# ntnu-arl/mimosa

Hardware: AMD Instinct MI355X
Metric: ICP corr+residual Mpts/sec, 131k-pt scan vs 5M-pt map, 1/2/4/8 GPU (higher is better)
Workload: dtype f64; 1 GPU; configs[1]: OS0-128 131072-pt scan vs 4963194-pt local map (511380 voxels, 2x5 rooms), k=5 point-to-plane, ENWIDE params, cold linearize per step; parallelism=single GPU, exact_fallback_queries=0

## Files before the change

mimosa_amd/csrc/icp_device.hpp:

```cpp
#pragma once

#include <hip/hip_runtime.h>

#include <cstdint>
#include <cstring>

#include "flagged_word.hpp"
#include "voxel_map.hpp"

namespace mh
{
constexpr int kPartialStride = 96;

struct MapView
{
  const int4 * table;
  const uint32_t * cells;
  const float4 * buckets;
  const uint4 * qbuckets;
  double inv_leaf;
  uint32_t mask;
  int n_off;
  int mode_idx;
};

struct DeviceResult
{
  double sums[kPartialStride];
  double eig_rot[9], eig_trans[9];
  double loc_comp[6];
  unsigned long long n_knn, n_cand, n_fallback, n_scanned;
  unsigned int status_hist[9];
};

constexpr int kLlSums = 96;
constexpr int kLlEig = 32;
constexpr int kLlRow = 8;
constexpr int kLocChunks = 4;
__host__ __device__ inline size_t ll_slot_words(int loc_grid_cap) { return static_cast<size_t>(kLlSums + kLlEig) + static_cast<size_t>(loc_grid_cap) * kLlRow; }

struct IcpArgs
{
  MapView map;
  const float4 * src;
  int n;
  int k;
  int cold;
  int use_huber;
  double R[9], t[3];
  double da_thresh, max_d2, plane_valid, sigma, huber;
  double inv_sigma;
  double inv_huber;
  double * q_da;
  double * mean;
  double * normal;
  int32_t * status;
  double * partials;
  unsigned int * ticket;
  unsigned int seq;
  int tail;
  uint4 * ll;
  unsigned long long * dbg;
  int reps;
  const uint32_t * n_dev = nullptr;
  double * shard_out = nullptr;
  double * rec = nullptr;
  int rec_n = 0;
};
__host__ __device__ inline size_t loc_record_bytes(size_t n) { return n * (6 * sizeof(double) + sizeof(int32_t)); }
constexpr int32_t kShardSkip = 0x100;

struct LocArgs
{
  unsigned int seq;
  int nv;
  const float4 * src;
  int n;
  int chunks_per_block;
  int k;
  int k3_blocks;
  uint4 * ll;
  double R[9];
  const double * normal;
  const int32_t * status;
  double * partials;
  unsigned int * ticket;
  const uint32_t * n_dev = nullptr;
  const double * sums = nullptr;
  double * shard_out = nullptr;
  const double * rec = nullptr;
  int rec_n = 0;
  unsigned long long * dbg = nullptr;
};

int linearize_class(int n, int k, bool shard, long long total = 0);
int class_grid(int n, int ppw);
int class_loc_grid(int n, int ppw, bool shard = false);
int linearize_grid_max(int n);
hipError_t launch_linearize(const IcpArgs & a, bool binary, hipStream_t stream);
hipError_t launch_localizability(const LocArgs & a, hipStream_t stream);
hipError_t launch_linearize_batch(const IcpArgs * d_args, const int * d_start, int n_factors, int total_grid, int tpb, int k,
                                  int n_off, bool binary, hipStream_t stream);
hipError_t launch_localizability_batch(const LocArgs * d_args, const int * d_start, int n_factors, int total_grid, int tpb,
                                       hipStream_t stream);
constexpr int kBatchInline = 8;
template <typename A>
struct BatchInline
{
  A a[kBatchInline];
  int start[kBatchInline + 1];
  int n;
  char pad[256];
};
template <typename A, typename ArgAt, typename GridAt>
inline int fill_batch_inline(BatchInline<A> & blk, int n, ArgAt && arg_at, GridAt && grid_at)
{
  std::memset(static_cast<void *>(&blk), 0, sizeof(blk));
  int acc = 0;
  for (int i = 0; i < n; ++i) {
    blk.a[i] = arg_at(i);
    blk.start[i] = acc;
    acc += grid_at(i);
  }
  blk.start[n] = acc;
  blk.n = n;
  return acc;
}
hipError_t launch_linearize_batch_inline(const BatchInline<IcpArgs> & blk, int total_grid, int tpb, int k, int n_off, bool binary,
                                         hipStream_t stream, bool shard = false);
hipError_t launch_localizability_batch_inline(const BatchInline<LocArgs> & blk, int total_grid, int tpb, hipStream_t stream, bool shard = false);
hipError_t launch_map_knn(const MapView & map, const double * q, int n, int k, double * pts, double * sq,
                          int32_t * found, hipStream_t stream);

size_t order_temp_bytes(int n);
hipError_t launch_spatial_order(const float4 * xyz_in, int n, float cell, uint32_t * keys2, uint32_t * vals, void * temp,
                                size_t temp_bytes, uint32_t * perm, float4 * xyz_out, hipStream_t stream);
size_t source_order_scratch_bytes(int n);
hipError_t launch_source_order(const mh_point32 * d_pts, int n, float cell, void * scratch, uint32_t * perm, float4 * xyz_out,
                               uint32_t * zero, int n_zero, hipStream_t stream);
hipError_t launch_unpermute_state(const uint32_t * perm, int n, const int32_t * st_in, const double * mean_in,
                                  const double * nrm_in, int32_t * st_out, double * mean_out, double * nrm_out,
                                  hipStream_t stream);

hipError_t launch_deskew(mh_point32 * pts, int n, const uint32_t * unique_ns, const float * Rt12, int n_groups,
// ... 7 lines not shown
```

mimosa_amd/csrc/icp_kernels.hip:

```cpp
#include <hip/hip_runtime.h>

#include <cstdlib>

#include "icp_device.hpp"

#ifndef MH_PRUNE_TRIPS
#define MH_PRUNE_TRIPS (trip == 1 || trip == 2)
#endif
#ifndef MH_PIPE
#define MH_PIPE 4
#endif
#ifndef MH_XCD_PIECES
#define MH_XCD_PIECES 2
#endif
#ifndef MH_PIPE_SMALL
#define MH_PIPE_SMALL 4
#endif
#include "map_device.hpp"
#include "math3.hpp"
#include "wave_dpp.hpp"

namespace mh
{
namespace
// ... 860 lines not shown
  jt[1] = -ns1;
  jt[2] = -ns2;
}

template <int K, bool BINARY, int NOFF, int TPB, bool SHARD, int QL = 1>
__device__ __forceinline__ void icp_linearize_body(const IcpArgs & a, const int block_id, const int n_blocks)
{
  static_assert(QL == 1 || (!SHARD && K == 5), "several lanes per query: plain k = 5 factors only");
  constexpr int PPW = TPB / QL;
  [[maybe_unused]] const bool lead = QL == 1 || (threadIdx.x & static_cast<unsigned int>(QL - 1)) == 0u;
  constexpr int NV = BINARY ? 13 : 7;
  constexpr int NENT = NV * (NV + 1) / 2;
  constexpr int EW = BINARY ? 96 : 32;
  constexpr int ROWW = NV;
  constexpr int kListWords = NOFF * PPW;
  constexpr int kFoldWords = (TPB / EW) * EW * 2 + EW * 2;
  constexpr int kArenaWords = kListWords > kFoldWords ? kListWords : kFoldWords;
  __shared__ __attribute__((aligned(16))) uint32_t s_arena[kArenaWords];
  __shared__ double s_tile[TPB * ROWW];
  __shared__ double s_wsum[(TPB / 64) * (NENT <= 32 ? 2 : 1) * NENT];
  __shared__ unsigned int s_cnt[4];
  __shared__ uint32_t s_scan[kScanLutWords];
  __shared__ bool s_last;

  uint32_t * s_list = s_arena + threadIdx.x / QL;
  double * s_aux = reinterpret_cast<double *>(s_arena);

#if !defined(MH_NO_INTERLEAVE)
  const int qi = [&] {
    if constexpr (QL > 1) return xcd_chunk(block_id, n_blocks) * PPW + static_cast<int>(threadIdx.x) / QL;
    constexpr int WPB = TPB / 64;
    const int cpx = n_blocks >> 3, x = block_id & 7, j = block_id >> 3, wv = static_cast<int>(threadIdx.x >> 6);
#if MH_XCD_PIECES > 1
    constexpr int P = MH_XCD_PIECES;
    static_assert(WPB % P == 0, "pieces must divide the waves of a workgroup");
    const int S = cpx * (WPB / P), p = wv / (WPB / P), o = (wv % (WPB / P)) * cpx + j;
    return ((p * 8 + ((p & 1) ? 7 - x : x)) * S + o) * 64 + static_cast<int>(threadIdx.x & 63u);
#else
    return ((x * cpx * WPB) + wv * cpx + j) * 64 + static_cast<int>(threadIdx.x & 63u);
#endif
  }();
#else
  const int qi = xcd_chunk(block_id, n_blocks) * PPW + static_cast<int>(threadIdx.x) / QL;
#endif
  const int k = (K == 5) ? 5 : a.k;
  const int n_pts = SHARD ? static_cast<int>(*a.n_dev) : a.n;
  float4 sp = make_float4(0.f, 0.f, 0.f, 0.f);
  if (qi < n_pts) sp = a.src[qi];
  if (threadIdx.x < 4) s_cnt[threadIdx.x] = 0u;
  fill_scan_lut<NOFF>(s_scan);
  __syncthreads();

  double row[NV];
  [[maybe_unused]] double rec_jr[3] = {0.0, 0.0, 0.0}, rec_jt[3] = {0.0, 0.0, 0.0};
  [[maybe_unused]] int rec_st = -1;
  uint32_t cnt_pack = 0u;
  bool did_knn = false, did_fall = false;
#ifdef MH_TIMELINE
  for (int rep = 0; rep < a.reps; ++rep) {
  if (rep > 0) {
    __syncthreads();
    if (threadIdx.x < 4) s_cnt[threadIdx.x] = 0u;
    __syncthreads();
  }
#endif
  MH_STAMP(a.dbg, 0);
#pragma unroll
  for (int j = 0; j < NV; ++j) row[j] = 0.0;

  if (qi < n_pts) {
    const double px = sp.x, py = sp.y, pz = sp.z;
    const double q0 = (a.R[0] * px + (a.R[1] * py + a.R[2] * pz)) + a.t[0];
    const double q1 = (a.R[3] * px + (a.R[4] * py + a.R[5] * pz)) + a.t[1];
    const double q2 = (a.R[6] * px + (a.R[7] * py + a.R[8] * pz)) + a.t[2];

    double qd0 = 0.0, qd1 = 0.0, qd2 = 0.0;
    int st = MH_UNPROCESSED;
    if (!a.cold) {
      qd0 = a.q_da[3 * qi + 0];
      qd1 = a.q_da[3 * qi + 1];
      qd2 = a.q_da[3 * qi + 2];
      st = a.status[qi];
    }
    bool gone = SHARD && (st & kShardSkip) != 0;
    if constexpr (SHARD) {
      if (a.cold) {
        const int raw = a.status[qi];
        gone = (raw & kShardSkip) != 0;
        if (gone && raw != -1) {
          a.status[qi] = kShardSkip;
          a.q_da[3 * qi + 0] = a.q_da[3 * qi + 1] = a.q_da[3 * qi + 2] = 0.0;
          a.mean[3 * qi + 0] = a.mean[3 * qi + 1] = a.mean[3 * qi + 2] = 0.0;
          a.normal[3 * qi + 0] = a.normal[3 * qi + 1] = a.normal[3 * qi + 2] = 0.0;
        }
      }
    }
    const double ddx = q0 - qd0, ddy = q1 - qd1, ddz = q2 - qd2;
    const bool update = !gone && (ddx * ddx + (ddy * ddy + ddz * ddz)) > a.da_thresh * a.da_thresh;

    double mean[3] = {0, 0, 0}, nrm[3] = {0, 0, 0};
    bool go = false;
    if (update) {
      st = MH_UNPROCESSED;
      if (lead) {
        a.q_da[3 * qi + 0] = q0;
        a.q_da[3 * qi + 1] = q1;
        a.q_da[3 * qi + 2] = q2;
      }
// ... 126 lines not shown
      }
    } else {
      if (!gone && st > MH_CORRES_PLANE_INVALID) {
        mean[0] = a.mean[3 * qi + 0];
        mean[1] = a.mean[3 * qi + 1];
        mean[2] = a.mean[3 * qi + 2];
        nrm[0] = a.normal[3 * qi + 0];
        nrm[1] = a.normal[3 * qi + 1];
        nrm[2] = a.normal[3 * qi + 2];
        go = true;
      } else if (a.cold && lead) {
        a.q_da[3 * qi + 0] = a.q_da[3 * qi + 1] = a.q_da[3 * qi + 2] = 0.0;
        a.mean[3 * qi + 0] = a.mean[3 * qi + 1] = a.mean[3 * qi + 2] = 0.0;
        a.normal[3 * qi + 0] = a.normal[3 * qi + 1] = a.normal[3 * qi + 2] = 0.0;
      }
    }

    if (go && lead) {
      double e = nrm[0] * (mean[0] - q0) + (nrm[1] * (mean[1] - q1) + nrm[2] * (mean[2] - q2));
      const double r2 = px * px + (py * py + pz * pz);
      const double e81 = 81.0 * (e * e);
      if (e81 * e81 > r2) {
        st = MH_MAX_ERROR;
      } else {
        double sw = 1.0;
        if (a.use_huber) {
          const double we = e * a.inv_sigma;
          if (fabs(we) > a.huber) sw = mh_rsqrt(fabs(we) * a.inv_huber);
        }
        const double wgt = sw * a.inv_sigma;
        e *= wgt;
        const double ns0 = a.R[0] * nrm[0] + (a.R[3] * nrm[1] + a.R[6] * nrm[2]);
        const double ns1 = a.R[1] * nrm[0] + (a.R[4] * nrm[1] + a.R[7] * nrm[2]);
        const double ns2 = a.R[2] * nrm[0] + (a.R[5] * nrm[1] + a.R[8] * nrm[2]);
        row[0] = (ns1 * pz - ns2 * py) * wgt;
        row[1] = (ns2 * px - ns0 * pz) * wgt;
        row[2] = (ns0 * py - ns1 * px) * wgt;
        row[3] = -ns0 * wgt;
        row[4] = -ns1 * wgt;
        row[5] = -ns2 * wgt;
        if constexpr (BINARY) {
          row[6] = (q1 * nrm[2] - q2 * nrm[1]) * wgt;
          row[7] = (q2 * nrm[0] - q0 * nrm[2]) * wgt;
          row[8] = (q0 * nrm[1] - q1 * nrm[0]) * wgt;
          row[9] = nrm[0] * wgt;
          row[10] = nrm[1] * wgt;
          row[11] = nrm[2] * wgt;
        }
        row[NV - 1] = e;
        st = MH_VALID;
      }
    }
    if (!gone && lead) a.status[qi] = st;
    if constexpr (!SHARD) {
      if (a.rec && lead) {
        if (st == MH_VALID) loc_directions(a, nrm[0], nrm[1], nrm[2], px, py, pz, rec_jr, rec_jt);
        rec_st = st;
      }
    }
  }
  {
    const uint32_t packed = wave_sum_to_lane63(cnt_pack);
    const unsigned long long mk = __ballot(did_knn), mf = __ballot(did_fall);
    if ((threadIdx.x & 63) == 63) {
      atomicAdd(&s_cnt[0], static_cast<unsigned int>(__popcll(mk)));
      atomicAdd(&s_cnt[1], packed & 0xFFFFu);
      atomicAdd(&s_cnt[2], static_cast<unsigned int>(__popcll(mf)));
      atomicAdd(&s_cnt[3], packed >> 16);
    }
    cnt_pack = 0u;
    did_knn = did_fall = false;
  }
#ifdef MH_TIMELINE
  }
#endif

  [[maybe_unused]] auto store_record = [&]() {
    if constexpr (!SHARD) {
      const size_t rn = static_cast<size_t>(a.rec_n);
      int32_t * rst = reinterpret_cast<int32_t *>(a.rec + 6 * rn);
#pragma unroll
      for (int c = 0; c < 3; ++c) {
        a.rec[static_cast<size_t>(c) * rn + qi] = rec_jr[c];
        a.rec[static_cast<size_t>(3 + c) * rn + qi] = rec_jt[c];
      }
      rst[qi] = rec_st;
    }
  };
  MH_STAMP(a.dbg, 3);
  {
    constexpr int WSEG = NENT <= 32 ? 2 : 1;
    constexpr int WPTS = 64 / WSEG;
    const int lane = static_cast<int>(threadIdx.x & 63u), wv = static_cast<int>(threadIdx.x >> 6);
    double * tile = s_tile + static_cast<size_t>(wv) * 64 * ROWW;
#pragma unroll
    for (int j = 0; j < NV; ++j) tile[lane * ROWW + j] = row[j];
    __builtin_amdgcn_fence(__ATOMIC_RELEASE, "wavefront");
    __builtin_amdgcn_wave_barrier();
    __builtin_amdgcn_fence(__ATOMIC_ACQUIRE, "wavefront");
    constexpr int ROUNDS = (NENT * WSEG + 63) / 64;
#pragma unroll
    for (int rd = 0; rd < ROUNDS; ++rd) {
      const int item = rd * 64 + lane;
      const int ent = WSEG == 2 ? (lane & 31) : item, seg = WSEG == 2 ? (lane >> 5) : 0;
      if (ent < NENT) {
        int r = 0, rem = ent;
        while (rem >= NV - r) {
          rem -= NV - r;
          ++r;
        }
        const int c = r + rem;
        const double * pr = tile + seg * WPTS * ROWW;
        double s0 = 0.0, s1 = 0.0, s2 = 0.0, s3 = 0.0;
#pragma unroll
        for (int p = 0; p < WPTS; p += 4) {
          s0 += pr[(p + 0) * ROWW + r] * pr[(p + 0) * ROWW + c];
          s1 += pr[(p + 1) * ROWW + r] * pr[(p + 1) * ROWW + c];
          s2 += pr[(p + 2) * ROWW + r] * pr[(p + 2) * ROWW + c];
          s3 += pr[(p + 3) * ROWW + r] * pr[(p + 3) * ROWW + c];
        }
        s_wsum[(wv * WSEG + seg) * NENT + ent] = (s0 + s1) + (s2 + s3);
      }
    }
    if constexpr (!SHARD) {
      if (a.rec && qi < a.n && lead) store_record();
    }
  }
  __syncthreads();
  MH_STAMP(a.dbg, 4);
  const bool fold_here = SHARD || a.tail != 0;
  const bool through = fold_here;
  if (threadIdx.x < NENT) {
    constexpr int NPART = (TPB / 64) * (NENT <= 32 ? 2 : 1);
    double pv[NPART];
#pragma unroll
    for (int g = 0; g < NPART; ++g) pv[g] = s_wsum[g * NENT + threadIdx.x];
    double s = 0.0;
#pragma unroll
    for (int g = 0; g < NPART; ++g) s += pv[g];
    double * dst = &a.partials[static_cast<size_t>(block_id) * kPartialStride + threadIdx.x];
    if (through)
      store_partial(dst, s);
    else
      *dst = s;
  }
  if (threadIdx.x >= 128 && threadIdx.x < 132) {
    double * dst = &a.partials[static_cast<size_t>(block_id) * kPartialStride + NENT + (threadIdx.x - 128)];
    const double c = static_cast<double>(s_cnt[threadIdx.x - 128]);
    if (through)
      store_partial(dst, c);
    else
      *dst = c;
  }

  MH_STAMP(a.dbg, 5);
  if (!fold_here) return;
  if (!arrive_is_last(a.ticket, static_cast<unsigned int>(n_blocks), &s_last)) return;
  MH_STAMP(a.dbg, 6);

  double * s_sum = s_aux + (TPB / EW) * EW;
  fold_rows<EW, TPB>(a.partials, n_blocks, NENT + 4, s_aux, s_sum);
  if constexpr (SHARD) {
    if (threadIdx.x < NENT + 4) a.shard_out[threadIdx.x] = s_sum[threadIdx.x];
  } else {
    if (threadIdx.x < NENT + 4) ll_store(a.ll + threadIdx.x, s_sum[threadIdx.x], a.seq);
  }
  MH_STAMP(a.dbg, 7);
}

template <int K, bool BINARY, int NOFF, int TPB, bool SHARD, int QL = 1>
__global__ __launch_bounds__(TPB) void icp_linearize_kernel(const IcpArgs a)
{
  icp_linearize_body<K, BINARY, NOFF, TPB, SHARD, QL>(a, static_cast<int>(blockIdx.x), static_cast<int>(gridDim.x));
}

template <typename T>
__device__ __forceinline__ T load_uniform(const T * p)
{
  static_assert(sizeof(T) % 4 == 0, "dword-sized argument blocks only");
// ... 4 lines not shown
    __device__ U() {}
  } u;
  const uint32_t * s = reinterpret_cast<const uint32_t *>(p);
  const int lane = static_cast<int>(threadIdx.x & 63u);
  uint32_t chunk[NL];
#pragma unroll
  for (int c = 0; c < NL; ++c) chunk[c] = s[c * 64 + lane];
#pragma unroll
  for (int i = 0; i < NW; ++i) u.w[i] = static_cast<uint32_t>(__builtin_amdgcn_readlane(static_cast<int>(chunk[i / 64]), i % 64));
  return u.v;
}

__device__ __forceinline__ int batch_factor_of(const int * start, int n_factors, int b)
{
  int f = 0;
  for (int i = 1; i < n_factors; ++i) f += (b >= start[i]) ? 1 : 0;
  return __builtin_amdgcn_readfirstlane(f);
}

template <int K, bool BINARY, int NOFF, int TPB>
__global__ __launch_bounds__(TPB) void icp_linearize_batch_kernel(const IcpArgs * args, const int * start, int n_factors)
{
  const int b = static_cast<int>(blockIdx.x);
  const int f = batch_factor_of(start, n_factors, b);
  const int s0 = __builtin_amdgcn_readfirstlane(start[f]), s1 = __builtin_amdgcn_readfirstlane(start[f + 1]);
  const IcpArgs a = load_uniform(args + f);
  icp_linearize_body<K, BINARY, NOFF, TPB, false>(a, b - s0, s1 - s0);
}

template <int NOFF, int QL>
__global__ __launch_bounds__(256) void icp_linearize_batch_ql_kernel(const IcpArgs * args, const int * start, int n_factors)
{
  const int b = static_cast<int>(blockIdx.x);
  const int f = batch_factor_of(start, n_factors, b);
  const int s0 = __builtin_amdgcn_readfirstlane(start[f]), s1 = __builtin_amdgcn_readfirstlane(start[f + 1]);
  const IcpArgs a = load_uniform(args + f);
  icp_linearize_body<5, false, NOFF, 256, false, QL>(a, b - s0, s1 - s0);
}

template <int K, bool BINARY, int NOFF, int TPB, bool SHARD, int QL = 1>
__global__ __launch_bounds__(TPB) void icp_linearize_batch_inline_kernel(const BatchInline<IcpArgs> blk)
{
  (void)blk;
  const auto * p = (const BatchInline<IcpArgs> *)__builtin_amdgcn_kernarg_segment_ptr();
  const int b = static_cast<int>(blockIdx.x);
  const int f = batch_factor_of(p->start, p->n, b);
  const int s0 = __builtin_amdgcn_readfirstlane(p->start[f]), s1 = __builtin_amdgcn_readfirstlane(p->start[f + 1]);
  const IcpArgs a = load_uniform(p->a + f);
  icp_linearize_body<K, BINARY, NOFF, TPB, SHARD, QL>(a, b - s0, s1 - s0);
}

__host__ __device__ constexpr int loc_tpb(int tpb, bool shard) { return (!shard && tpb > 256) ? 256 : tpb; }
__host__ __device__ constexpr int loc_threads(int tpb, bool shard) { return loc_tpb(tpb, shard) + (shard ? 0 : 64); }
#ifndef MH_LOC_BLOCKS_512
#define MH_LOC_BLOCKS_512 2
#endif
__host__ __device__ constexpr int loc_ch(int tpb, bool shard) { return shard ? 1 : (tpb > 256 ? 2 * MH_LOC_BLOCKS_512 : kLocChunks); }

template <int TPB, bool SHARD, int CH, bool XW = false>
__device__ __forceinline__ void icp_localizability_body(const LocArgs & a, const int block_id, const int n_blocks)
{
  constexpr int NW = TPB / 64;
  const bool worker = !XW || threadIdx.x < static_cast<unsigned int>(TPB);
  __shared__ double s_w[NW][16];
  __shared__ double s_seg[TPB + 96 + 96];

  const int lane = threadIdx.x & 63, wv = threadIdx.x >> 6;
  MH_STAMP4(a.dbg, 0);
  double v[6] = {0, 0, 0, 0, 0, 0};
  unsigned long long hpack = 0ull;
  const int n_pts = !worker ? 0 : (SHARD ? static_cast<int>(*a.n_dev) : (a.rec ? a.n : 0));
  int st_c[CH];
  double jr_c[CH][3], jt_c[CH][3];
  [[maybe_unused]] float4 sp_c[CH];
  [[maybe_unused]] double nx_c[CH], ny_c[CH], nz_c[CH];
  auto load_chunk = [&](const int ch) {
    const int i = (block_id * CH + ch) * TPB + static_cast<int>(threadIdx.x);
    const int i_ld = i < n_pts ? i : 0;
    st_c[ch] = -1;
    jr_c[ch][0] = jr_c[ch][1] = jr_c[ch][2] = jt_c[ch][0] = jt_c[ch][1] = jt_c[ch][2] = 0.0;
    if constexpr (SHARD) {
      sp_c[ch] = make_float4(0.f, 0.f, 0.f, 0.f);
      nx_c[ch] = ny_c[ch] = nz_c[ch] = 0.0;
      if (n_pts > 0) {
        st_c[ch] = a.status[i_ld];
        sp_c[ch] = a.src[i_ld];
        nx_c[ch] = a.normal[3 * i_ld];
        ny_c[ch] = a.normal[3 * i_ld + 1];
        nz_c[ch] = a.normal[3 * i_ld + 2];
      }
    } else if (n_pts > 0) {
      const size_t rn = static_cast<size_t>(a.rec_n);
      const int32_t * rst = reinterpret_cast<const int32_t *>(a.rec + 6 * rn);
      st_c[ch] = rst[i_ld];
#pragma unroll
      for (int c = 0; c < 3; ++c) {
        jr_c[ch][c] = a.rec[static_cast<size_t>(c) * rn + i_ld];
        jt_c[ch][c] = a.rec[static_cast<size_t>(3 + c) * rn + i_ld];
      }
    }
    if (i >= n_pts) st_c[ch] = -1;
  };
  auto load_all = [&]() {
    MH_STAMP4(a.dbg, 1);
#pragma unroll
    for (int ch = 0; ch < CH; ++ch) load_chunk(ch);
  };
  const double * sums = nullptr;
  double * s_h = s_seg + TPB;
  if constexpr (SHARD) {
    sums = a.sums;
  } else {
    const int n_ent = a.nv * (a.nv + 1) / 2 + 4;
    constexpr int FB = 32;
    if (a.nv == 7)
      fold_rows<32, TPB, true, FB>(a.partials, a.k3_blocks, n_ent, s_seg, s_h);
    else
      fold_rows<96, TPB, true, FB>(a.partials, a.k3_blocks, n_ent, s_seg, s_h);
    sums = s_h;
  }
  load_all();
  MH_STAMP4(a.dbg, 2);
  __shared__ double s_E[18];
  if (XW ? (threadIdx.x == TPB || threadIdx.x == TPB + 1) : (threadIdx.x == TPB - 64 || threadIdx.x == TPB - 128)) {
    const int NV = a.nv, o = (XW ? threadIdx.x == TPB + 1 : threadIdx.x == TPB - 64) ? 3 : 0;
    double Hb[9];
    for (int r = 0; r < 3; ++r)
      for (int c = 0; c < 3; ++c) {
        const int rr = (r < c ? r : c) + o, cc = (r < c ? c : r) + o;
        Hb[3 * r + c] = sums[rr * NV - rr * (rr - 1) / 2 + (cc - rr)];
      }
    double loc[3], E[9];
    if (!sym_eigvec3_fast(Hb, E)) compute_localizability(Hb, loc, E);
    for (int q = 0; q < 9; ++q) s_E[(o ? 9 : 0) + q] = E[q];
  }
  MH_STAMP4(a.dbg, 3);
  if constexpr (SHARD) {
#pragma unroll
    for (int ch = 0; ch < CH; ++ch)
      loc_directions(a, nx_c[ch], ny_c[ch], nz_c[ch], static_cast<double>(sp_c[ch].x), static_cast<double>(sp_c[ch].y),
                     static_cast<double>(sp_c[ch].z), jr_c[ch], jt_c[ch]);
  }
  MH_STAMP4(a.dbg, 4);
  __syncthreads();
  MH_STAMP4(a.dbg, 5);
  double er[9], et[9];
#pragma unroll
  for (int q = 0; q < 9; ++q) {
    er[q] = s_E[q];
    et[q] = s_E[9 + q];
  }
#pragma unroll
  for (int ch = 0; ch < CH; ++ch) {
    const int st = st_c[ch];
    if (st == MH_VALID) {
#pragma unroll
      for (int c = 0; c < 3; ++c) {
        const double tc = fabs(jt_c[ch][0] * et[c] + (jt_c[ch][1] * et[3 + c] + jt_c[ch][2] * et[6 + c]));
        const double rc = fabs(jr_c[ch][0] * er[c] + (jr_c[ch][1] * er[3 + c] + jr_c[ch][2] * er[6 + c]));
        v[c] += tc >= 0.5 ? tc : 0.0;
        v[3 + c] += rc >= 0.5 ? rc : 0.0;
      }
    }
    hpack += st >= 0 && st < 9 ? (1ull << (4 * st)) : 0ull;
  }
  MH_STAMP4(a.dbg, 6);
  wave_sum6_f64_to_lane63(v);
  uint32_t hw[3];
#pragma unroll
  for (int g = 0; g < 3; ++g) {
    const uint32_t f0 = static_cast<uint32_t>(hpack >> (12 * g)) & 15u, f1 = static_cast<uint32_t>(hpack >> (12 * g + 4)) & 15u,
                   f2 = static_cast<uint32_t>(hpack >> (12 * g + 8)) & 15u;
    hw[g] = f0 | (f1 << 10) | (f2 << 20);
  }
  wave_sum3_to_lane63(hw);
  if (lane == 63 && worker) {
#pragma unroll
    for (int j = 0; j < 6; ++j) s_w[wv][j] = v[j];
#pragma unroll
    for (int g = 0; g < 3; ++g) {
      s_w[wv][6 + 3 * g + 0] = static_cast<double>(hw[g] & 1023u);
      s_w[wv][6 + 3 * g + 1] = static_cast<double>((hw[g] >> 10) & 1023u);
      s_w[wv][6 + 3 * g + 2] = static_cast<double>((hw[g] >> 20) & 1023u);
    }
  }
  MH_STAMP4(a.dbg, 7);
  __syncthreads();
  MH_STAMP4(a.dbg, 8);
  if constexpr (!SHARD) {
    uint4 * ll_rows = a.ll + (kLlSums + kLlEig) + static_cast<size_t>(block_id) * kLlRow;
    if (threadIdx.x < 6) {
      double s = 0.0;
      for (int w2 = 0; w2 < NW; ++w2) s += s_w[w2][threadIdx.x];
      ll_store(ll_rows + threadIdx.x, s, a.seq);
    } else if (threadIdx.x < 8) {
      const int h0 = threadIdx.x == 6 ? 0 : 5, hn = threadIdx.x == 6 ? 5 : 4;
      unsigned long long pk = 0ull;
      for (int h = 0; h < hn; ++h) {
        unsigned int c = 0u;
        for (int w2 = 0; w2 < NW; ++w2) c += static_cast<unsigned int>(s_w[w2][6 + h0 + h]);
        pk |= static_cast<unsigned long long>(c) << (12 * h);
      }
      ll_store_bits(ll_rows + threadIdx.x, pk, a.seq);
    }
    if (block_id == 0) {
      const int n_ent = a.nv * (a.nv + 1) / 2 + 4;
      if (threadIdx.x >= 64 && static_cast<int>(threadIdx.x) < 64 + n_ent) ll_store(a.ll + (threadIdx.x - 64), s_h[threadIdx.x - 64], a.seq);
      if (threadIdx.x >= 192 && threadIdx.x < 192 + 18) ll_store(a.ll + kLlSums + (threadIdx.x - 192), s_E[threadIdx.x - 192], a.seq);
    }
#ifdef MH_TIMELINE
    asm volatile("s_waitcnt vmcnt(0)" ::: "memory");
#endif
// ... 349 lines not shown
```

mimosa_amd/csrc/mh_api.hip:

```cpp
#include <hip/hip_runtime.h>

#include <atomic>
#include <cmath>
#include <cstdio>
#include <cstdlib>
#include <cstring>
#include <ctime>
#include <mutex>
#include <new>
#include <unordered_map>
#include <string>
#include <vector>

#include "../../include/mimosa_hip.h"
#include "align_device.hpp"
#include "icp_device.hpp"
#include "math3.hpp"
#include "mh_internal.hpp"
#include "scan_device.hpp"
#include "shard_device.hpp"
#include "voxel_map.hpp"

namespace
{
// ... 427 lines not shown
{
  if (!src || !out) return fail(src ? src->ctx : nullptr, MH_ERR_INVALID_ARG, "mh_icp_clone: NULL argument");
  *out = nullptr;
  mh_ctx * ctx = src->ctx;
  if (src->n_pending) return fail(ctx, MH_ERR_INVALID_ARG, "mh_icp_clone: source has linearize calls in flight");
  MH_HIP(ctx, mh_enter(ctx));
  mh_icp * icp = new (std::nothrow) mh_icp;
  if (!icp) return fail(ctx, MH_ERR_OOM, "mh_icp_clone: host allocation failed");
  icp->ctx = ctx;
  icp->map = src->map;
  mh_map_retain(icp->map);
  map_add_reader(icp->map, ctx);
  icp->n = src->n;
  icp->cfg = src->cfg;
  icp->binary = src->binary;
  int rc = icp_alloc(icp);
  if (rc != MH_OK) {
    mh_icp_destroy(icp);
    return rc;
  }
  const size_t n = src->n;
  auto cp = [&](const DevBuf & a, DevBuf & b, size_t bytes) {
    return bytes ? hipMemcpyAsync(b.p, a.p, bytes, hipMemcpyDeviceToDevice, ctx->stream) : hipSuccess;
  };
  MH_HIP(ctx, cp(src->d_src, icp->d_src, n * sizeof(float4)));
  MH_HIP(ctx, cp(src->d_qda, icp->d_qda, n * 3 * sizeof(double)));
  MH_HIP(ctx, cp(src->d_mean, icp->d_mean, n * 3 * sizeof(double)));
  MH_HIP(ctx, cp(src->d_normal, icp->d_normal, n * 3 * sizeof(double)));
  MH_HIP(ctx, cp(src->d_status, icp->d_status, n * sizeof(int32_t)));
  if (src->ordered) {
    MH_HIP(ctx, icp->d_perm.reserve(n * sizeof(uint32_t), ctx->stream, false));
    MH_HIP(ctx, cp(src->d_perm, icp->d_perm, n * sizeof(uint32_t)));
    icp->ordered = true;
  }
  MH_HIP(ctx, hipMemsetAsync(icp->d_ticket.p, 0, 2 * sizeof(unsigned int), ctx->stream));
  MH_HIP(ctx, hipStreamSynchronize(ctx->stream));
  icp->cold = src->cold;
  icp->components = src->components;
  icp->linearize_count = src->linearize_count;
  *out = icp;
  return MH_OK;
}
int mh_icp_clone(const mh_icp * src, mh_icp ** out)
{
  return guarded(src ? src->ctx : nullptr, "mh_icp_clone", [&]() -> int { return mh_icp_clone_impl(src, out); });
}

void mh_icp_destroy(mh_icp * icp)
{
  if (!icp) return;
  (void)mh_enter(icp->ctx);
  (void)hipStreamSynchronize(icp->ctx->stream);
  if (icp->in_window && icp->ctx->window.active) window_release(icp->ctx);
  icp->d_rec.release(true);
  icp->d_src.release(true);
  icp->d_qda.release(true);
  icp->d_mean.release(true);
  icp->d_normal.release(true);
  icp->d_status.release(true);
  icp->d_partials.release(true);
  icp->d_ticket.release(true);
  icp->d_dbg.release(true);
  icp->d_perm.release(true);
  for (DevBuf * b : {&icp->d_origin, &icp->x_src, &icp->x_qda, &icp->x_mean, &icp->x_normal, &icp->x_status, &icp->x_origin, &icp->s_keys_a,
                     &icp->s_keys_b, &icp->s_idx_a, &icp->s_idx_b, &icp->s_counts, &icp->s_temp, &icp->d_sums})
    b->release(true);
  if (icp->h_counts) (void)hipHostFree(icp->h_counts);
  if (icp->h_ll) AllocCache::free_pinned(icp->h_ll, icp->ll_words * sizeof(uint4) * kMaxPending);
  icp->d_align.release(true);
  if (icp->h_align) AllocCache::free_pinned(icp->h_align, kAlignStageBytes);
  if (icp->events_ready)
    for (auto & ev : icp->events)
      for (auto & e : ev) (void)hipEventDestroy(e);
  if (icp->map) {
    map_remove_reader(icp->map, icp->ctx);
    mh_map_release(icp->map);
  }
  delete icp;
}

size_t mh_icp_size(const mh_icp * icp) { return icp ? icp->n : 0; }

#ifdef MH_TIMELINE
int mh_icp_timeline(mh_icp * icp, unsigned long long * out, size_t capacity_words, size_t * n_words)
{
  if (!icp || !out || !n_words) return MH_ERR_INVALID_ARG;
  mh_ctx * ctx = icp->ctx;
  const size_t words = 2 * static_cast<size_t>(mh::linearize_grid_max(static_cast<int>(icp->n))) * 8 * 16;
  *n_words = words;
  if (capacity_words < words) return MH_ERR_INVALID_ARG;
  MH_HIP(ctx, mh_enter(ctx));
  MH_HIP(ctx, hipStreamSynchronize(ctx->stream));
  MH_HIP(ctx, hipMemcpy(out, icp->d_dbg.p, words * sizeof(unsigned long long), hipMemcpyDeviceToHost));
  return MH_OK;
}
#endif

static int mh_icp_reset_impl(mh_icp * icp)
{
  if (!icp) return fail(nullptr, MH_ERR_INVALID_ARG, "mh_icp_reset: icp is NULL");
  if (icp->in_window) return fail(icp->ctx, MH_ERR_INVALID_ARG, "mh_icp_reset: the factor is in a window call in flight");
  if (icp->align.active) return fail(icp->ctx, MH_ERR_INVALID_ARG, "mh_icp_reset: an alignment is in flight");
  icp->cold = true;
  return MH_OK;
}
int mh_icp_reset(mh_icp * icp)
{
// ... 15 lines not shown
struct LinearizeTxn
{
  mh_icp * icp;
  bool cold = true, committed = false;
  int count = 0, pending = 0;
  explicit LinearizeTxn(mh_icp * i) : icp(i)
  {
    if (icp) {
      cold = icp->cold;
      count = icp->linearize_count;
      pending = icp->n_pending;
    }
  }
  LinearizeTxn(LinearizeTxn && o) noexcept : icp(o.icp), cold(o.cold), committed(o.committed), count(o.count), pending(o.pending) { o.icp = nullptr; }
  LinearizeTxn(const LinearizeTxn &) = delete;
  LinearizeTxn & operator=(const LinearizeTxn &) = delete;
  void commit() { committed = true; }
  ~LinearizeTxn()
  {
    if (icp && !committed) {
      icp->cold = cold;
      icp->linearize_count = count;
      icp->n_pending = pending;
    }
  }
};

static unsigned int next_call_seq()
{
  static std::atomic<unsigned int> counter{0};
  unsigned int v = counter.fetch_add(1u, std::memory_order_relaxed) + 1u;
  if (v == 0u) v = counter.fetch_add(1u, std::memory_order_relaxed) + 1u;
  return v;
}

static int linearize_prepare(mh_icp * icp, const double R_src[9], const double t_src[3], const double * R_tgt,
                             const double * t_tgt, const double g_unit[3], mh_icp_result * out, bool allow_timing,
                             mh::IcpArgs & a, mh::LocArgs & l, bool & timed)
{
  if (!icp || !R_src || !t_src || !g_unit || !out)
    return fail(icp ? icp->ctx : nullptr, MH_ERR_INVALID_ARG, "mh_icp_linearize: NULL argument");
  mh_ctx * ctx = icp->ctx;
  if (icp->binary && (!R_tgt || !t_tgt)) return fail(ctx, MH_ERR_INVALID_ARG, "mh_icp_linearize: binary factor needs the target pose");
  if (icp->n_pending >= kMaxPending) return fail(ctx, MH_ERR_INVALID_ARG, "mh_icp_linearize_async: too many calls in flight");
  MH_HIP(ctx, mh_enter(ctx));
  if (ctx->profiling && !icp->events_ready) {
    for (auto & ev : icp->events)
      for (auto & e : ev) MH_HIP(ctx, hipEventCreate(&e));
    icp->events_ready = true;
  }

  const size_t row_doubles = static_cast<size_t>(mh::linearize_grid_max(static_cast<int>(icp->n ? icp->n : 1))) * mh::kPartialStride;
  MH_HIP(ctx, icp->d_partials.reserve(row_doubles * sizeof(double), ctx->stream, false));
  a.rec = nullptr;
  a.rec_n = 0;
  if (icp->components && icp->n > 0) {
    MH_HIP(ctx, icp->d_rec.reserve(mh::loc_record_bytes(icp->n), ctx->stream, false));
    a.rec = static_cast<double *>(icp->d_rec.p);
    a.rec_n = static_cast<int>(icp->n);
  }
  a.map = map_view(icp->map);
  a.src = static_cast<const float4 *>(icp->d_src.p);
  a.n = static_cast<int>(icp->n);
  a.k = static_cast<int>(icp->cfg.num_corres_points);
  a.cold = icp->cold ? 1 : 0;
  a.use_huber = icp->cfg.use_huber;
  pose_inverse_compose(R_src, t_src, icp->binary ? R_tgt : nullptr, icp->binary ? t_tgt : nullptr, a.R, a.t);
  a.da_thresh = static_cast<double>(icp->cfg.target_ivox_map_min_dist_in_voxel / 4);
  a.max_d2 = static_cast<double>(icp->cfg.max_corres_distance * icp->cfg.max_corres_distance);
  a.plane_valid = static_cast<double>(icp->cfg.plane_validity_distance);
  a.sigma = static_cast<double>(icp->cfg.lidar_point_noise_std_dev);
  a.inv_sigma = 1.0 / a.sigma;
  a.huber = static_cast<double>(icp->cfg.huber_threshold);
  a.inv_huber = 1.0 / a.huber;
  a.q_da = static_cast<double *>(icp->d_qda.p);
  a.mean = static_cast<double *>(icp->d_mean.p);
  a.normal = static_cast<double *>(icp->d_normal.p);
  a.status = static_cast<int32_t *>(icp->d_status.p);
  a.partials = static_cast<double *>(icp->d_partials.p);
  a.ticket = static_cast<unsigned int *>(icp->d_ticket.p);
  a.dbg = static_cast<unsigned long long *>(icp->d_dbg.p);
  a.reps = 1;
#ifdef MH_TIMELINE
  if (const char * rp = std::getenv("MH_REPS")) a.reps = std::atoi(rp);
#endif

  l.src = a.src;
  l.seq = 0;
  l.nv = icp->binary ? 13 : 7;
  l.n = a.n;
  l.k = a.k;
  l.chunks_per_block = 1;
  std::memcpy(l.R, a.R, sizeof(l.R));
  l.normal = a.normal;
  l.status = a.status;
  l.partials = a.partials;
  l.ticket = a.ticket + 1;
  l.rec = a.rec;
  l.rec_n = a.rec_n;
#ifdef MH_TIMELINE
  l.dbg = a.dbg ? a.dbg + static_cast<size_t>(mh::linearize_grid_max(static_cast<int>(icp->n ? icp->n : 1))) * 8 * 16 : nullptr;
#endif

  const int slot = icp->n_pending;
  PendingCall & pc = icp->pending[slot];
  pc.out = out;
  std::memcpy(pc.R, a.R, sizeof(pc.R));
  for (int i = 0; i < 3; ++i) pc.gz[i] = -g_unit[i];
  pc.linearize_count = ++icp->linearize_count;
  timed = allow_timing && ctx->profiling > 0 && (pc.linearize_count % ctx->profiling) == 0;
  if (timed) {
    for (int i = 0; i < 3; ++i) pc.ev[i] = icp->events[slot][i];
  } else {
    pc.ev[0] = pc.ev[1] = pc.ev[2] = nullptr;
  }
  pc.seq = 0;
  pc.components = icp->components;
  pc.seq_has_basis = false;
  pc.loc_blocks = 0;
  pc.launched_k4 = false;
  a.seq = 0;
  a.tail = 1;
  a.ll = l.ll = nullptr;
  const int ppw = mh::linearize_class(a.n, a.k, false);
  l.k3_blocks = mh::class_grid(a.n, ppw);
  if (a.n > 0) {
    pc.seq = a.seq = l.seq = next_call_seq();
    a.ll = l.ll = icp->d_h_ll + static_cast<size_t>(slot) * icp->ll_words;
    pc.loc_blocks = mh::class_loc_grid(a.n, ppw);
  }
  icp->n_pending++;
  icp->cold = false;
  return MH_OK;
}

static int linearize_enqueue(mh_icp * icp, const double R_src[9], const double t_src[3], const double * R_tgt,
                             const double * t_tgt, const double g_unit[3], mh_icp_result * out)
{
  mh::IcpArgs a;
  mh::LocArgs l;
  bool timed = false;
  LinearizeTxn txn(icp);
  const int rc = linearize_prepare(icp, R_src, t_src, R_tgt, t_tgt, g_unit, out, true, a, l, timed);
  if (rc != MH_OK) return rc;
  mh_ctx * ctx = icp->ctx;
  const int slot = icp->n_pending - 1;
  PendingCall & pc = icp->pending[slot];
  if (timed) MH_HIP(ctx, hipEventRecord(pc.ev[0], ctx->stream));
  if (a.n > 0) {
    a.tail = pc.components ? 0 : 1;
    const double tl0 = g_wt.on ? WaitTrace::now() : 0.0;
    MH_HIP(ctx, mh::launch_linearize(a, icp->binary, ctx->stream));
// ... 308 lines not shown
}

static bool align_read_row(const mh_icp * icp, int i, long spin_ns, double * row)
{
  const uint4 * base = icp->h_ll + static_cast<size_t>(i) * icp->ll_words + mh::kLlSums;
  mh::SpinBudget spin(spin_ns);
  for (int w = mh::kRowWords - 1; w >= 0; --w)
    if (!spin.until([&] { return mh::ll_read(reinterpret_cast<const uint64_t *>(base + w), icp->align.seq[i], row[w]); })) return false;
  return true;
}

static int align_wait_row(mh_icp * icp, int i, double * row)
{
  mh_ctx * ctx = icp->ctx;
  if (align_read_row(icp, i, 50000000L, row)) return MH_OK;
  MH_HIP(ctx, hipStreamSynchronize(ctx->stream));
  if (align_read_row(icp, i, 2000000L, row)) return MH_OK;
  return fail(ctx, MH_ERR_HIP, "mh_icp_align: the stream drained without the chain's results");
}

static void align_abandon(mh_icp * icp)
{
  (void)hipStreamSynchronize(icp->ctx->stream);
  icp->align.active = false;
  icp->n_pending = 0;
}

static int align_begin(mh_icp * icp, const double R0[9], const double t0[3], const double g_unit[3], const mh_icp_align_config * cfg,
                       mh_icp_align_result * out)
{
  if (!icp || !R0 || !t0 || !g_unit || !cfg || !out) return fail(icp ? icp->ctx : nullptr, MH_ERR_INVALID_ARG, "mh_icp_align: NULL argument");
  mh_ctx * ctx = icp->ctx;
  if (icp->binary) return fail(ctx, MH_ERR_UNSUPPORTED, "mh_icp_align: unary factors only");
  if (icp->n_pending || icp->align.active) return fail(ctx, MH_ERR_INVALID_ARG, "mh_icp_align: the factor has calls in flight");
  if (cfg->max_iters < 1 || cfg->max_iters > kMaxPending) return fail(ctx, MH_ERR_INVALID_ARG, "mh_icp_align: max_iters must be in 1..64");
  if (!(cfg->eps_rot >= 0.0) || !(cfg->eps_trans >= 0.0) || !(cfg->damping >= 0.0) || !(cfg->prior_sigma_rot >= 0.0) ||
      !(cfg->prior_sigma_trans >= 0.0) || cfg->check_every < 0)
    return fail(ctx, MH_ERR_INVALID_ARG, "mh_icp_align: eps, damping, prior sigmas and check_every must be >= 0");
  if (icp->no_order || icp->cap_n > icp->n) return fail(ctx, MH_ERR_UNSUPPORTED, "mh_icp_align: not for the factors of the map-sharded path");
  if (icp->n == 0) return fail(ctx, MH_ERR_INVALID_ARG, "mh_icp_align: the factor has no points");
  MH_HIP(ctx, mh_enter(ctx));
  MH_HIP(ctx, icp->d_align.reserve(kAlignBytes, ctx->stream, false));
  if (!icp->h_align) MH_HIP(ctx, AllocCache::alloc_pinned(&icp->h_align, kAlignStageBytes));

  mh::IcpArgs a;
  {
    mh::LocArgs l;
    bool timed = false;
    mh_icp_result scratch;
    LinearizeTxn txn(icp);
    const int rc = linearize_prepare(icp, R0, t0, nullptr, nullptr, g_unit, &scratch, false, a, l, timed);
    if (rc != MH_OK) return rc;
  }
  a.rec = nullptr;
  a.rec_n = 0;
  a.tail = 1;

  mh_icp::AlignCall & c = icp->align;
  c.cfg = *cfg;
  c.out = out;
  std::memcpy(c.R0, R0, sizeof(c.R0));
  for (int i = 0; i < 3; ++i) c.gz[i] = -g_unit[i];
  c.queued = 0;
  c.count0 = icp->linearize_count;
  c.cold0 = icp->cold;
  mh::AlignParams & p = c.p;
  for (int i = 0; i < 3; ++i) p.gz[i] = c.gz[i];
  p.eps_rot = cfg->eps_rot;
  p.eps_trans = cfg->eps_trans;
  p.damping = cfg->damping;
  p.prior_rot = cfg->prior_sigma_rot > 0.0 ? 1.0 / (cfg->prior_sigma_rot * cfg->prior_sigma_rot) : 0.0;
  p.prior_trans = cfg->prior_sigma_trans > 0.0 ? 1.0 / (cfg->prior_sigma_trans * cfg->prior_sigma_trans) : 0.0;
  p.thresh_rot = icp->cfg.degen_thresh_rot;
  p.thresh_trans = icp->cfg.degen_thresh_trans;
  p.reg_4_dof = icp->cfg.reg_4_dof;
  p.project_on_degeneracy = icp->cfg.project_on_degneneracy;

  char * h = static_cast<char *>(icp->h_align);
  char * d = static_cast<char *>(icp->d_align.p);
  const int ppw = mh::linearize_class(a.n, a.k, false);
  int * start = reinterpret_cast<int *>(h);
  start[0] = 0;
  start[1] = mh::class_grid(a.n, ppw);
  mh::AlignState st;
  std::memset(&st, 0, sizeof(st));
  std::memcpy(st.R, a.R, sizeof(st.R));
  std::memcpy(st.t, a.t, sizeof(st.t));
  std::memcpy(h + 64, &st, sizeof(st));
  auto * blocks = reinterpret_cast<mh::IcpArgs *>(h + kAlignBlocksAt);
  for (int i = 0; i < cfg->max_iters; ++i) {
    mh::IcpArgs b = a;
    b.cold = (i == 0 && c.cold0) ? 1 : 0;
    b.seq = c.seq[i] = next_call_seq();
    b.ll = reinterpret_cast<uint4 *>(d + kAlignLlAt) + static_cast<size_t>(i) * kAlignLlWords;
    blocks[i] = b;
  }
  MH_HIP(ctx, hipMemcpyAsync(d, h, kAlignBlocksAt + sizeof(mh::IcpArgs) * static_cast<size_t>(cfg->max_iters), hipMemcpyHostToDevice, ctx->stream));
  c.active = true;
  icp->n_pending = kMaxPending;
  return MH_OK;
}

static int align_enqueue(mh_icp * icp, int upto)
{
  mh_ctx * ctx = icp->ctx;
  mh_icp::AlignCall & c = icp->align;
  char * d = static_cast<char *>(icp->d_align.p);
  auto * blocks = reinterpret_cast<mh::IcpArgs *>(d + kAlignBlocksAt);
// ... 194 lines not shown
    std::memset(ctx->h_window_rows, 0, kWinRowWords * sizeof(uint4) * kMaxPending);
    MH_HIP(ctx, hipHostGetDevicePointer(reinterpret_cast<void **>(&ctx->d_window_rows), ctx->h_window_rows, 0));
  }

  WindowCall & c = ctx->window;
  c.W = static_cast<int>(W);
  c.iters = cfg->iters;
  c.queued = 0;
  c.out = out;
  c.trace_poses = trace_poses;
  c.relin = relin != nullptr;
  c.relin_rot = relin ? relin->relin_rot : 0.0;
  c.relin_trans = relin ? relin->relin_trans : 0.0;
  c.evaluated_mask = evaluated_mask;
  for (int i = 0; i < 3; ++i) c.gz[i] = -g_unit[i];
  const std::vector<LaunchGroup> groups = window_launch_groups(icps, W);
  c.launches.clear();
  c.n_slots = 0;
  for (size_t f = 0; f < W; ++f) c.slot[f] = -1;
  for (const LaunchGroup & g : groups) {
    WindowLaunch wl{g.tpb, g.k, g.n_off, c.n_slots, static_cast<int>(g.members.size()), 0};
    for (size_t f : g.members) c.slot[f] = c.n_slots++;
    c.launches.push_back(wl);
  }

  char * h = static_cast<char *>(ctx->h_window);
  char * d = static_cast<char *>(ctx->d_window);
  auto * blocks = reinterpret_cast<mh::IcpArgs *>(h + kWinBlocksAt);
  mh::WindowState st;
  std::memset(&st, 0, sizeof(st));
  for (int it = 0; it < cfg->iters; ++it) c.seq[it] = next_call_seq();
  for (size_t f = 0; f < W; ++f) {
    mh_icp * icp = icps[f];
    c.icps[f] = icp;
    c.count0[f] = icp->linearize_count;
    std::memcpy(c.R0[f], R + 9 * f, sizeof(c.R0[f]));
    std::memcpy(st.R[f], R + 9 * f, sizeof(st.R[f]));
    std::memcpy(st.t[f], t + 3 * f, sizeof(st.t[f]));
    if ((zmask >> f) & 1u) {
      std::memcpy(st.ZR[f], Z_R + 9 * f, sizeof(st.ZR[f]));
      std::memcpy(st.Zt[f], Z_t + 3 * f, sizeof(st.Zt[f]));
    }
    if (icp->n == 0) continue;
    mh::IcpArgs a;
    const bool cold0 = icp->cold;
    {
      mh::LocArgs l;
      bool timed = false;
      mh_icp_result scratch;
      LinearizeTxn txn(icp);
      const int rc = linearize_prepare(icp, R + 9 * f, t + 3 * f, nullptr, nullptr, g_unit, &scratch, false, a, l, timed);
      if (rc != MH_OK) return rc;
    }
    a.rec = nullptr;
    a.rec_n = 0;
    a.tail = 1;
    a.ll = reinterpret_cast<uint4 *>(d + kWinLlAt) + 32 * f;
    std::memcpy(st.R[f], a.R, sizeof(st.R[f]));
    std::memcpy(st.t[f], a.t, sizeof(st.t[f]));
    for (int it = 0; it < cfg->iters; ++it) {
      mh::IcpArgs b = a;
      b.cold = (it == 0 && cold0) ? 1 : 0;
      b.seq = c.seq[it];
      blocks[static_cast<size_t>(it) * c.n_slots + c.slot[f]] = b;
    }
  }
  int * prefix = reinterpret_cast<int *>(h);
  for (size_t gi = 0; gi < c.launches.size(); ++gi) {
    WindowLaunch & wl = c.launches[gi];
    int * start = prefix + wl.first + static_cast<int>(gi);
    int acc = 0;
    for (int i = 0; i < wl.n; ++i) {
      start[i] = acc;
      acc += mh::class_grid(blocks[wl.first + i].n, wl.tpb);
    }
    start[wl.n] = acc;
    wl.grid = acc;
  }
  std::memcpy(h + kWinStateAt, &st, sizeof(st));

  mh::WindowParams & p = c.p;
  std::memset(&p, 0, sizeof(p));
  p.W = c.W;
  p.has_Z = zmask;
  for (size_t f = 0; f < W; ++f) {
    const mh_icp * icp = icps[f];
    if (icp->n) p.have |= 1u << f;
    if (icp->cfg.reg_4_dof) p.reg_4_dof |= 1u << f;
    if (icp->cfg.project_on_degneneracy) p.project_on_degeneracy |= 1u << f;
    p.thresh_rot[f] = icp->cfg.degen_thresh_rot;
    p.thresh_trans[f] = icp->cfg.degen_thresh_trans;
  }
  for (int i = 0; i < 3; ++i) p.gz[i] = c.gz[i];
  for (int i = 0; i < 6; ++i) {
    p.Wb[i] = cfg->between_info[i];
    p.prior[i] = cfg->prior_info[i];
  }
  p.damping = cfg->damping;
  p.eps_rot = cfg->eps_rot;
  p.eps_trans = cfg->eps_trans;

  MH_HIP(ctx, hipMemcpyAsync(d, h, kWinBlocksAt + sizeof(mh::IcpArgs) * static_cast<size_t>(c.n_slots) * static_cast<size_t>(cfg->iters), hipMemcpyHostToDevice, ctx->stream));
  c.active = true;
  for (size_t f = 0; f < W; ++f) {
    icps[f]->in_window = true;
    icps[f]->n_pending = kMaxPending;
  }
  return MH_OK;
// ... 924 lines not shown
```

mimosa_amd/csrc/mh_internal.hpp:

```cpp
#pragma once

#include <chrono>
#include <cstdio>
#include <cstdlib>
#include <hip/hip_runtime.h>

#include <cstdint>
#include <cstring>
#include <mutex>
#include <set>
#include <new>
#include <string>
#include <unordered_map>
#include <utility>
#include <vector>

#include "../../include/mimosa_hip.h"
#include <atomic>

#include "align_device.hpp"
#include "window_device.hpp"
#include "icp_device.hpp"
#include "map_device.hpp"
#include "scan_device.hpp"
// ... 519 lines not shown
}
inline hipError_t map_wait_readers(mh_map * m)
{
  std::vector<hipStream_t> streams;
  {
    std::lock_guard<std::mutex> g(m->readers_mu);
    for (const auto & r : m->readers)
      if (r.second > 0 && r.first != m->ctx) streams.push_back(r.first->stream);
  }
  for (hipStream_t st : streams) {
    const hipError_t e = hipStreamSynchronize(st);
    if (e != hipSuccess) return e;
  }
  return hipSuccess;
}

inline mh::MapView map_view(const mh_map * m)
{
  mh::MapView v;
  v.table = static_cast<const int4 *>(m->d_table.p);
  v.cells = static_cast<const uint32_t *>(m->d_cells.p);
  v.buckets = static_cast<const float4 *>(m->d_buckets.p);
  v.qbuckets = static_cast<const uint4 *>(m->d_qbuckets.p);
  v.inv_leaf = m->inv_leaf;
  v.mask = static_cast<uint32_t>(m->table_cap - 1);
  v.n_off = m->n_off;
  v.mode_idx = m->n_off == 1 ? 0 : (m->n_off == 7 ? 1 : (m->n_off == 19 ? 2 : 3));
  return v;
}

struct PendingCall
{
  mh_icp_result * out;
  double R[9];
  double gz[3];
  int parity;
  int linearize_count;
  unsigned int seq;
  bool components;
  bool seq_has_basis = false;
  int loc_blocks = 0;
  bool launched_k4 = false;
  hipEvent_t ev[3];
};

struct mh_icp
{
  mh_ctx * ctx;
  mh_map * map;
  size_t n;
  mh_reg_config cfg;
  bool binary;
  DevBuf d_src, d_qda, d_mean, d_normal, d_status, d_partials, d_ticket, d_dbg, d_perm;
  DevBuf d_rec;
  bool ordered = false;
  uint4 * h_ll = nullptr;
  uint4 * d_h_ll = nullptr;
  size_t ll_words = 0;
  PendingCall pending[kMaxPending];
  int n_pending = 0;
  int parity = 0;
  bool cold = true;
  bool components = true;
  int linearize_count = 0;
  hipEvent_t events[kMaxPending][3];
  bool events_ready = false;
  unsigned int seq_counter = 0;
  bool no_order = false;
  size_t cap_n = 0;
  DevBuf d_origin, x_src, x_qda, x_mean, x_normal, x_status, x_origin;
  DevBuf s_keys_a, s_keys_b, s_idx_a, s_idx_b, s_counts, s_temp, d_sums;
  uint32_t * h_counts = nullptr;
  bool origin_ready = false, plan_open = false;
  uint32_t n_movers = 0;
  DevBuf d_align;
  void * h_align = nullptr;
  struct AlignCall
  {
    bool active = false;
    mh_icp_align_config cfg{};
    mh_icp_align_result * out = nullptr;
    double R0[9], gz[3];
    int queued = 0, count0 = 0;
    bool cold0 = true;
    unsigned int seq[kMaxPending];
    mh::AlignParams p;
  } align;
  bool in_window = false;
};

inline void window_release(mh_ctx * ctx)
{
  WindowCall & c = ctx->window;
  for (int i = 0; i < c.W; ++i) {
    c.icps[i]->in_window = false;
    c.icps[i]->n_pending = 0;
  }
  c.active = false;
}

struct LaunchGroup
{
  int tpb, k, n_off;
  bool binary;
  std::vector<size_t> members;
  int first = 0, grid = 0, grid4 = 0;
};
// ... 12 lines not shown
```

Baseline: 3207 Mpts/s.

## Recompute localizability directions in loc kernel instead of recording per-point Jacobians

Removes the per-point record buffer that the linearize kernel filled with rotation/translation Jacobian directions and status for the localizability kernel. The localizability kernel now reloads status, source point and normal and recomputes the directions itself, using fma in the non-shard path. This drops the 6-double store per point from linearize and the record reads, at the cost of extra loads and arithmetic in the loc kernel. The loc chunk count also changes from 4 to 2 and the 512-thread special case is removed.

```diff
diff --git a/mimosa_amd/csrc/icp_device.hpp b/mimosa_amd/csrc/icp_device.hpp
--- a/mimosa_amd/csrc/icp_device.hpp
+++ b/mimosa_amd/csrc/icp_device.hpp
@@ -36,7 +36,10 @@
 constexpr int kLlSums = 96;
 constexpr int kLlEig = 32;
 constexpr int kLlRow = 8;
-constexpr int kLocChunks = 4;
+#ifndef MH_LOC_CHUNKS
+#define MH_LOC_CHUNKS 2
+#endif
+constexpr int kLocChunks = MH_LOC_CHUNKS;
 __host__ __device__ inline size_t ll_slot_words(int loc_grid_cap) { return static_cast<size_t>(kLlSums + kLlEig) + static_cast<size_t>(loc_grid_cap) * kLlRow; }
 
 struct IcpArgs
@@ -64,10 +67,7 @@
   int reps;
   const uint32_t * n_dev = nullptr;
   double * shard_out = nullptr;
-  double * rec = nullptr;
-  int rec_n = 0;
 };
-__host__ __device__ inline size_t loc_record_bytes(size_t n) { return n * (6 * sizeof(double) + sizeof(int32_t)); }
 constexpr int32_t kShardSkip = 0x100;
 
 struct LocArgs
@@ -88,8 +88,7 @@
   const uint32_t * n_dev = nullptr;
   const double * sums = nullptr;
   double * shard_out = nullptr;
-  const double * rec = nullptr;
-  int rec_n = 0;
+  int comps = 1;
   unsigned long long * dbg = nullptr;
 };
 
diff --git a/mimosa_amd/csrc/icp_kernels.hip b/mimosa_amd/csrc/icp_kernels.hip
--- a/mimosa_amd/csrc/icp_kernels.hip
+++ b/mimosa_amd/csrc/icp_kernels.hip
@@ -936,8 +936,6 @@
   __syncthreads();
 
   double row[NV];
-  [[maybe_unused]] double rec_jr[3] = {0.0, 0.0, 0.0}, rec_jt[3] = {0.0, 0.0, 0.0};
-  [[maybe_unused]] int rec_st = -1;
   uint32_t cnt_pack = 0u;
   bool did_knn = false, did_fall = false;
 #ifdef MH_TIMELINE
@@ -1170,12 +1168,6 @@
       }
     }
     if (!gone && lead) a.status[qi] = st;
-    if constexpr (!SHARD) {
-      if (a.rec && lead) {
-        if (st == MH_VALID) loc_directions(a, nrm[0], nrm[1], nrm[2], px, py, pz, rec_jr, rec_jt);
-        rec_st = st;
-      }
-    }
   }
   {
     const uint32_t packed = wave_sum_to_lane63(cnt_pack);
@@ -1193,18 +1185,6 @@
   }
 #endif
 
-  [[maybe_unused]] auto store_record = [&]() {
-    if constexpr (!SHARD) {
-      const size_t rn = static_cast<size_t>(a.rec_n);
-      int32_t * rst = reinterpret_cast<int32_t *>(a.rec + 6 * rn);
-#pragma unroll
-      for (int c = 0; c < 3; ++c) {
-        a.rec[static_cast<size_t>(c) * rn + qi] = rec_jr[c];
-        a.rec[static_cast<size_t>(3 + c) * rn + qi] = rec_jt[c];
-      }
-      rst[qi] = rec_st;
-    }
-  };
   MH_STAMP(a.dbg, 3);
   {
     constexpr int WSEG = NENT <= 32 ? 2 : 1;
@@ -1240,9 +1220,6 @@
         s_wsum[(wv * WSEG + seg) * NENT + ent] = (s0 + s1) + (s2 + s3);
       }
     }
-    if constexpr (!SHARD) {
-      if (a.rec && qi < a.n && lead) store_record();
-    }
   }
   __syncthreads();
   MH_STAMP(a.dbg, 4);
@@ -1353,10 +1330,7 @@
 
 __host__ __device__ constexpr int loc_tpb(int tpb, bool shard) { return (!shard && tpb > 256) ? 256 : tpb; }
 __host__ __device__ constexpr int loc_threads(int tpb, bool shard) { return loc_tpb(tpb, shard) + (shard ? 0 : 64); }
-#ifndef MH_LOC_BLOCKS_512
-#define MH_LOC_BLOCKS_512 2
-#endif
-__host__ __device__ constexpr int loc_ch(int tpb, bool shard) { return shard ? 1 : (tpb > 256 ? 2 * MH_LOC_BLOCKS_512 : kLocChunks); }
+__host__ __device__ constexpr int loc_ch(int tpb, bool shard) { return shard ? 1 : kLocChunks; }
 
 template <int TPB, bool SHARD, int CH, bool XW = false>
 __device__ __forceinline__ void icp_localizability_body(const LocArgs & a, const int block_id, const int n_blocks)
@@ -1370,35 +1344,24 @@
   MH_STAMP4(a.dbg, 0);
   double v[6] = {0, 0, 0, 0, 0, 0};
   unsigned long long hpack = 0ull;
-  const int n_pts = !worker ? 0 : (SHARD ? static_cast<int>(*a.n_dev) : (a.rec ? a.n : 0));
+  const int n_pts = !worker ? 0 : (SHARD ? static_cast<int>(*a.n_dev) : (a.comps ? a.n : 0));
   int st_c[CH];
   double jr_c[CH][3], jt_c[CH][3];
-  [[maybe_unused]] float4 sp_c[CH];
-  [[maybe_unused]] double nx_c[CH], ny_c[CH], nz_c[CH];
+  float4 sp_c[CH];
+  double nx_c[CH], ny_c[CH], nz_c[CH];
   auto load_chunk = [&](const int ch) {
     const int i = (block_id * CH + ch) * TPB + static_cast<int>(threadIdx.x);
     const int i_ld = i < n_pts ? i : 0;
     st_c[ch] = -1;
     jr_c[ch][0] = jr_c[ch][1] = jr_c[ch][2] = jt_c[ch][0] = jt_c[ch][1] = jt_c[ch][2] = 0.0;
-    if constexpr (SHARD) {
-      sp_c[ch] = make_float4(0.f, 0.f, 0.f, 0.f);
-      nx_c[ch] = ny_c[ch] = nz_c[ch] = 0.0;
-      if (n_pts > 0) {
-        st_c[ch] = a.status[i_ld];
-        sp_c[ch] = a.src[i_ld];
-        nx_c[ch] = a.normal[3 * i_ld];
-        ny_c[ch] = a.normal[3 * i_ld + 1];
-        nz_c[ch] = a.normal[3 * i_ld + 2];
-      }
-    } else if (n_pts > 0) {
-      const size_t rn = static_cast<size_t>(a.rec_n);
-      const int32_t * rst = reinterpret_cast<const int32_t *>(a.rec + 6 * rn);
-      st_c[ch] = rst[i_ld];
-#pragma unroll
-      for (int c = 0; c < 3; ++c) {
-        jr_c[ch][c] = a.rec[static_cast<size_t>(c) * rn + i_ld];
-        jt_c[ch][c] = a.rec[static_cast<size_t>(3 + c) * rn + i_ld];
-      }
+    sp_c[ch] = make_float4(0.f, 0.f, 0.f, 0.f);
+    nx_c[ch] = ny_c[ch] = nz_c[ch] = 0.0;
+    if (n_pts > 0) {
+      st_c[ch] = a.status[i_ld];
+      sp_c[ch] = a.src[i_ld];
+      nx_c[ch] = a.normal[3 * i_ld];
+      ny_c[ch] = a.normal[3 * i_ld + 1];
+      nz_c[ch] = a.normal[3 * i_ld + 2];
     }
     if (i >= n_pts) st_c[ch] = -1;
   };
@@ -1436,12 +1399,10 @@
     for (int q = 0; q < 9; ++q) s_E[(o ? 9 : 0) + q] = E[q];
   }
   MH_STAMP4(a.dbg, 3);
-  if constexpr (SHARD) {
-#pragma unroll
-    for (int ch = 0; ch < CH; ++ch)
-      loc_directions(a, nx_c[ch], ny_c[ch], nz_c[ch], static_cast<double>(sp_c[ch].x), static_cast<double>(sp_c[ch].y),
-                     static_cast<double>(sp_c[ch].z), jr_c[ch], jt_c[ch]);
-  }
+#pragma unroll
+  for (int ch = 0; ch < CH; ++ch)
+    loc_directions(a, nx_c[ch], ny_c[ch], nz_c[ch], static_cast<double>(sp_c[ch].x), static_cast<double>(sp_c[ch].y),
+                   static_cast<double>(sp_c[ch].z), jr_c[ch], jt_c[ch]);
   MH_STAMP4(a.dbg, 4);
   __syncthreads();
   MH_STAMP4(a.dbg, 5);
@@ -1457,8 +1418,14 @@
     if (st == MH_VALID) {
 #pragma unroll
       for (int c = 0; c < 3; ++c) {
-        const double tc = fabs(jt_c[ch][0] * et[c] + (jt_c[ch][1] * et[3 + c] + jt_c[ch][2] * et[6 + c]));
-        const double rc = fabs(jr_c[ch][0] * er[c] + (jr_c[ch][1] * er[3 + c] + jr_c[ch][2] * er[6 + c]));
+        double tc, rc;
+        if constexpr (SHARD) {
+          tc = fabs(jt_c[ch][0] * et[c] + (jt_c[ch][1] * et[3 + c] + jt_c[ch][2] * et[6 + c]));
+          rc = fabs(jr_c[ch][0] * er[c] + (jr_c[ch][1] * er[3 + c] + jr_c[ch][2] * er[6 + c]));
+        } else {
+          tc = fabs(fma(jt_c[ch][0], et[c], fma(jt_c[ch][1], et[3 + c], jt_c[ch][2] * et[6 + c])));
+          rc = fabs(fma(jr_c[ch][0], er[c], fma(jr_c[ch][1], er[3 + c], jr_c[ch][2] * er[6 + c])));
+        }
         v[c] += tc >= 0.5 ? tc : 0.0;
         v[3 + c] += rc >= 0.5 ? rc : 0.0;
       }
diff --git a/mimosa_amd/csrc/mh_api.hip b/mimosa_amd/csrc/mh_api.hip
--- a/mimosa_amd/csrc/mh_api.hip
+++ b/mimosa_amd/csrc/mh_api.hip
@@ -503,7 +503,6 @@
   (void)mh_enter(icp->ctx);
   (void)hipStreamSynchronize(icp->ctx->stream);
   if (icp->in_window && icp->ctx->window.active) window_release(icp->ctx);
-  icp->d_rec.release(true);
   icp->d_src.release(true);
   icp->d_qda.release(true);
   icp->d_mean.release(true);
@@ -625,13 +624,6 @@
 
   const size_t row_doubles = static_cast<size_t>(mh::linearize_grid_max(static_cast<int>(icp->n ? icp->n : 1))) * mh::kPartialStride;
   MH_HIP(ctx, icp->d_partials.reserve(row_doubles * sizeof(double), ctx->stream, false));
-  a.rec = nullptr;
-  a.rec_n = 0;
-  if (icp->components && icp->n > 0) {
-    MH_HIP(ctx, icp->d_rec.reserve(mh::loc_record_bytes(icp->n), ctx->stream, false));
-    a.rec = static_cast<double *>(icp->d_rec.p);
-    a.rec_n = static_cast<int>(icp->n);
-  }
   a.map = map_view(icp->map);
   a.src = static_cast<const float4 *>(icp->d_src.p);
   a.n = static_cast<int>(icp->n);
@@ -669,8 +661,7 @@
   l.status = a.status;
   l.partials = a.partials;
   l.ticket = a.ticket + 1;
-  l.rec = a.rec;
-  l.rec_n = a.rec_n;
+  l.comps = icp->components ? 1 : 0;
 #ifdef MH_TIMELINE
   l.dbg = a.dbg ? a.dbg + static_cast<size_t>(mh::linearize_grid_max(static_cast<int>(icp->n ? icp->n : 1))) * 8 * 16 : nullptr;
 #endif
@@ -1085,8 +1076,6 @@
     const int rc = linearize_prepare(icp, R0, t0, nullptr, nullptr, g_unit, &scratch, false, a, l, timed);
     if (rc != MH_OK) return rc;
   }
-  a.rec = nullptr;
-  a.rec_n = 0;
   a.tail = 1;
 
   mh_icp::AlignCall & c = icp->align;
@@ -1387,8 +1376,6 @@
       const int rc = linearize_prepare(icp, R + 9 * f, t + 3 * f, nullptr, nullptr, g_unit, &scratch, false, a, l, timed);
       if (rc != MH_OK) return rc;
     }
-    a.rec = nullptr;
-    a.rec_n = 0;
     a.tail = 1;
     a.ll = reinterpret_cast<uint4 *>(d + kWinLlAt) + 32 * f;
     std::memcpy(st.R[f], a.R, sizeof(st.R[f]));
diff --git a/mimosa_amd/csrc/mh_internal.hpp b/mimosa_amd/csrc/mh_internal.hpp
--- a/mimosa_amd/csrc/mh_internal.hpp
+++ b/mimosa_amd/csrc/mh_internal.hpp
@@ -595,7 +595,6 @@
   mh_reg_config cfg;
   bool binary;
   DevBuf d_src, d_qda, d_mean, d_normal, d_status, d_partials, d_ticket, d_dbg, d_perm;
-  DevBuf d_rec;
   bool ordered = false;
   uint4 * h_ll = nullptr;
   uint4 * d_h_ll = nullptr;
```

New measurement: 3094 Mpts/s. 0.965x the previous value.
